# YuemingJin/STswinCL

Measured on AMD Instinct MI355X. Metric: input frames/s, TswinPlus fwd+bwd+Adam, 4-frame 512x512 clips, higher is better.
Workload: dtype bf16; 1 GPU; BASELINE.json configs[1]: TswinPlus(12) seg train step, 4 clips/GPU x T=4 frames x 3x512x512, swin res (64,64), OHEM-CE, Adam; T=4 because the reference asserts it (swin_512.py:313); clips_per_gpu=4, frames_per_clip=4, parallelism=dp1, graph_requested=True

## Files before the change

include/stswin_hip.h:

```cpp
#ifndef STSWIN_HIP_H
#define STSWIN_HIP_H
#ifdef __cplusplus
extern "C" {
#endif

#define STSWIN_GF_GELU 1
#define STSWIN_GF_RESID 2
#define STSWIN_GF_MUL_DGELU 4
#define STSWIN_GF_OUT_F32 8
#define STSWIN_GF_ACCUM 16
#define STSWIN_GF_RELU 32
#define STSWIN_GF_MUL_R 8192
#define STSWIN_GF_C2_DGELU 16384
#define STSWIN_GF_CS_PARTIAL 32768
#define STSWIN_GF_CS_SQ 65536
#define STSWIN_GF_TAPSKIP (1 << 29)
#define STSWIN_GF_BIG 128
#define STSWIN_GF_MID 512
#define STSWIN_GF_NOPIPE 1024
#define STSWIN_GF_HALF 2048
#define STSWIN_GF_M32PP (1u << 31)
#define STSWIN_GF_W4R (1 << 30)
#define STSWIN_GF_ROT 4096
#define STSWIN_GF_NOBIG 256
// ... 35 lines not shown
                       void* stream);
long stswin_conv3x3_c64_wgrad_scratch(int frames, int H, int W);
int stswin_conv3x3_c64_wgrad(const void* dy, const void* x, float* dw, int tapminor, int accumulate, float* scratch, long scratch_floats,
                             int frames, int H, int W, void* stream);

int stswin_gemm_nt(int dtype, const void* A, long lda, const int* a_rows, const void* B, long ldb, void* C, long ldc,
                   const int* c_rows, void* C2, long ldc2, const float* bias, const void* R, long ldr,
                   const int* r_rows, int M, int N, int Kseg, int S, float scale, int scale_cols, int flags,
                   float* colsum , void* stream);
int stswin_cs_reduce(const float* partials, int M, int N, float* out, void* stream);
#define STSWIN_TN_OVERWRITE (1 << 27)
#define STSWIN_TN_NO_COMBINE (1 << 26)
long stswin_gemm_nt_splitk_scratch(int M, int N, int Kseg, int S);
int stswin_gemm_nt_splitk(const void* A, long lda, const int* a_rows, const void* B, long ldb, void* C, long ldc, const float* bias, int M, int N,
                          int Kseg, int S, int relu, float* workspace, long workspace_floats, void* stream);
int stswin_tn_fused_hold(int delta);
int stswin_set_cu_budget(int cus);
int stswin_gemm_tn(int dtype, const void* At, long lda, const int* at_rows, const void* Bt, long ldb, const int* bt_rows,
                   float* C, long ldc, int Mk, int Ni, int Nj, int splits, int bseg,
                   float* workspace , long workspace_floats, void* stream);
#define STSWIN_TN_GROUP_DECLINED (-1050)
typedef struct stswin_tn_problem {
  const void* At; long lda; const int* at_rows;
  const void* Bt; long ldb; const int* bt_rows;
  float* C; long ldc;
  int Mk, Ni, Nj, bseg;
  int overwrite;
  int tapminor;
} stswin_tn_problem;
int stswin_gemm_tn_group(int dtype, int count, const stswin_tn_problem* problems, float* workspace, long workspace_floats, int* splits_out,
                         void* stream);
int stswin_tn_combine(const float* workspace, float* C, long ldc, int Ni, int Nj, int splits, int overwrite, int slab_bf16,
                      void* stream);
#define STSWIN_VAR_F32 100
#define STSWIN_VAR_NT_RING256_REGEPI 1
#define STSWIN_VAR_NT_RING256_LDSEPI 2
#define STSWIN_VAR_NT_RING256_NOPIPE 3
#define STSWIN_VAR_NT_RING256_W4 14
#define STSWIN_VAR_NT_STREAM 4
#define STSWIN_VAR_NT_DUO 5
#define STSWIN_VAR_NT_RING256x128_PP 6
#define STSWIN_VAR_NT_MID 7
#define STSWIN_VAR_NT_256x64 8
#define STSWIN_VAR_NT_128x64 9
#define STSWIN_VAR_NT_128x128 10
#define STSWIN_VAR_NT_128x128_W4 11
#define STSWIN_VAR_NT_SPLITK 13
#define STSWIN_VAR_NT_ROWS 12
#define STSWIN_VAR_TN_RING_PLAIN 20
#define STSWIN_VAR_TN_RING_ATROWS 21
#define STSWIN_VAR_TN_RING_BTROWS 22
#define STSWIN_VAR_TN_RING_BSEG 23
#define STSWIN_VAR_TN_128x128 30
#define STSWIN_VAR_TN_128x128_W4 31
#define STSWIN_VAR_TN_ROWS 32
#define STSWIN_VAR_TN_SLABS_F32 0x1000
#define STSWIN_VAR_TN_SLABS_BF16 0x2000
#define STSWIN_VAR_TN_FUSED 0x8000
#define STSWIN_VAR_TN_TAPMINOR 0x4000
#define STSWIN_TN_OUT_TAPMINOR (1 << 25)
int stswin_gemm_nt_qkv_fp8(const void* A, long lda, const int* a_rows, const void* B, long ldb, void* out8, long ld8, float* scales,
                           long ld_scales, const float* bias, int M, int N, int Kseg, float scale, int scale_cols, int rows_per_problem,
                           int head_dim, void* stream);
int stswin_win_attn_fwd_f8(const void* qkv8, long ld8, const float* scales, long ld_scales, void* out, long ldo, const float* biasT,
                           const float* maskT, int nB_, int nW, int T_frames, int ws, int heads, int C, int bias_windows,
                           const int* bias_index, void* stream);
// ... 232 lines not shown
```

stswincl_amd/csrc/gemm.hip:

```cpp
#include "common.h"
#include "stswin_hip.h"
#include <cstdint>
#include <cstdlib>
#include <type_traits>

enum {
  GF_GELU = STSWIN_GF_GELU, GF_RESID = STSWIN_GF_RESID, GF_MUL_DGELU = STSWIN_GF_MUL_DGELU, GF_OUT_F32 = STSWIN_GF_OUT_F32,
  GF_ACCUM = STSWIN_GF_ACCUM, GF_RELU = STSWIN_GF_RELU, GF_MUL_R = STSWIN_GF_MUL_R, GF_C2_DGELU = STSWIN_GF_C2_DGELU,
  GF_CS_PARTIAL = STSWIN_GF_CS_PARTIAL, GF_CS_SQ = STSWIN_GF_CS_SQ, GF_TAPSKIP = STSWIN_GF_TAPSKIP,
  GF_WAVES4 = STSWIN_GF_WAVES4, GF_BIG = STSWIN_GF_BIG, GF_NOBIG = STSWIN_GF_NOBIG, GF_MID = STSWIN_GF_MID, GF_NOPIPE = STSWIN_GF_NOPIPE,
  GF_HALF = STSWIN_GF_HALF, GF_ROT = STSWIN_GF_ROT, GF_NOREGEPI = STSWIN_GF_NOREGEPI, GF_NOSTREAM = STSWIN_GF_NOSTREAM,
  GF_DUO = STSWIN_GF_DUO, GF_STREAM = STSWIN_GF_STREAM, GF_NONARROW = STSWIN_GF_NONARROW, GF_NODEEP = STSWIN_GF_NODEEP,
  GF_DEEP = STSWIN_GF_DEEP, GF_W4R = STSWIN_GF_W4R, GF_M32PP = (int)STSWIN_GF_M32PP,
};

#ifdef STSWIN_TUNING
#define STSWIN_DBG(flags, bit) (((flags) & (1 << (bit))) != 0)
#else
#define STSWIN_DBG(flags, bit) false
#endif
enum { GF_DEBUG_BITS = (1 << 17) | (1 << 18) | (1 << 19) | (1 << 20) | (1 << 21) };
#ifdef STSWIN_TUNING
static __device__ int g_dbg_stagger[2] = {8, 0};
extern "C" int stswin_debug_set_stagger(int phases, int ticks) {
// ... 1600 lines not shown
      for (int u = 0; u < 8; ++u) v[u] = *(const bf16x8*)(src + (long)(s + u) * total);
#pragma unroll
      for (int u = 0; u < 8; ++u)
#pragma unroll
        for (int e = 0; e < 8; ++e) a[e] += (float)v[u][e];
    }
    for (; s < splits; ++s) {
      const bf16x8 v = *(const bf16x8*)(src + (long)s * total);
#pragma unroll
      for (int e = 0; e < 8; ++e) a[e] += (float)v[e];
    }
    if (perm > 0) {
      const int S = Nj / perm, sg = j / perm, c = j - sg * perm;
      float* d = C + (long)i * ldc + (long)c * S + sg;
#pragma unroll
      for (int e = 0; e < 8; ++e) d[(long)e * S] = overwrite ? a[e] : d[(long)e * S] + a[e];
      return;
    }
    float* dst = C + (long)i * ldc + j;
    if ((ldc & 3) == 0) {
      f32x4 lo = {a[0], a[1], a[2], a[3]}, hi = {a[4], a[5], a[6], a[7]};
      if (!overwrite) { lo += *(const f32x4*)dst; hi += *(const f32x4*)(dst + 4); }
      *(f32x4*)dst = lo;
      *(f32x4*)(dst + 4) = hi;
    } else {
      for (int e = 0; e < 8; ++e) dst[e] = overwrite ? a[e] : dst[e] + a[e];
    }
    return;
  }
  const long idx = ((long)blockIdx.x * 256 + threadIdx.x) * 4;
  if (idx >= (long)Ni * Nj) return;
  const int i = idx / Nj, j = idx % Nj;
  f32x4 a = {0.f, 0.f, 0.f, 0.f};
  for (int s = 0; s < splits; ++s) a += *(const f32x4*)(slabs + (long)s * Ni * Nj + idx);
  if (perm > 0) {
    const int S = Nj / perm, sg = j / perm, c = j - sg * perm;
    float* d = C + (long)i * ldc + (long)c * S + sg;
#pragma unroll
    for (int e = 0; e < 4; ++e) d[(long)e * S] = overwrite ? a[e] : d[(long)e * S] + a[e];
    return;
  }
  float* dst = C + (long)i * ldc + j;
  if (overwrite) {
    if ((ldc & 3) == 0) *(f32x4*)dst = a;
    else { for (int e = 0; e < 4; ++e) dst[e] = a[e]; }
  } else if ((ldc & 3) == 0) { *(f32x4*)dst = *(const f32x4*)dst + a; }
  else { for (int e = 0; e < 4; ++e) dst[e] += a[e]; }
}

static thread_local int g_last_variant[2] = {0, 0};
extern "C" int stswin_tuning_build() {
#ifdef STSWIN_TUNING
  return 1;
#else
  return 0;
#endif
}
extern "C" int stswin_last_variant(int family) { return family >= 0 && family < 2 ? g_last_variant[family] : -1; }

static int set_lds_once(const void* fn) {
  return (int)hipFuncSetAttribute(fn, hipFuncAttributeMaxDynamicSharedMemorySize, 65536);
}

extern "C" int stswin_cs_reduce(const float* partials, int M, int N, float* out, void* stream) {
  if (M <= 0 || N <= 0) return 0;
  if (N % 4) return -1004;
  const int rows = 2 * ((M + 255) / 256);
// ... 716 lines not shown
  dim3 grid(((Ni + 127) / 128) * ((Nj + 127) / 128) * splits);
  static int once = set_lds_once((const void*)gemm_tn_kernel<bf16, 4>) | set_lds_once((const void*)gemm_tn_kernel<float, 4>) |
                    set_lds_once((const void*)gemm_tn_kernel<bf16, 8>) | set_lds_once((const void*)gemm_tn_kernel<float, 8>);
  (void)once;
  const bool w8 = splits_flags_w4 == 0;
  g_last_variant[1] = ((w8 ? STSWIN_VAR_TN_128x128 : STSWIN_VAR_TN_128x128_W4) + (dtype ? STSWIN_VAR_F32 : 0)) |
                      (use_slabs ? (slab_bf16 ? STSWIN_VAR_TN_SLABS_BF16 : STSWIN_VAR_TN_SLABS_F32) : 0) | ((use_slabs && perm) ? 0x4000 : 0) |
                      (splits << 16);
  if (dtype == 0) {
    if (w8) hipLaunchKernelGGL((gemm_tn_kernel<bf16, 8>), grid, dim3(512), 65536, (hipStream_t)stream, p);
    else hipLaunchKernelGGL((gemm_tn_kernel<bf16, 4>), grid, dim3(256), 65536, (hipStream_t)stream, p);
  } else {
    if (w8) hipLaunchKernelGGL((gemm_tn_kernel<float, 8>), grid, dim3(512), 65536, (hipStream_t)stream, p);
    else hipLaunchKernelGGL((gemm_tn_kernel<float, 4>), grid, dim3(256), 65536, (hipStream_t)stream, p);
  }
  if (use_slabs && !no_combine) {
    const long n4 = slab_bf16 ? ((long)Ni * Nj + 7) / 8 : ((long)Ni * Nj + 3) / 4;
    hipLaunchKernelGGL(tn_reduce_kernel, dim3((unsigned)((n4 + 255) / 256)), dim3(256), 0, (hipStream_t)stream, workspace, C, ldc,
                       Ni, Nj, splits, overwrite, slab_bf16, perm);
  }
  STSWIN_CHECK_LAUNCH();
  return 0;
}

extern "C" int stswin_tn_combine(const float* workspace, float* C, long ldc, int Ni, int Nj, int splits, int overwrite, int slab_bf16,
                                 void* stream) {
  if (!workspace || !C || Ni <= 0 || Nj <= 0 || splits < 2) return -1007;
  const long n4 = slab_bf16 ? ((long)Ni * Nj + 7) / 8 : ((long)Ni * Nj + 3) / 4;
  hipLaunchKernelGGL(tn_reduce_kernel, dim3((unsigned)((n4 + 255) / 256)), dim3(256), 0, (hipStream_t)stream, workspace, C, ldc, Ni, Nj,
                     splits, overwrite, slab_bf16, 0);
  STSWIN_CHECK_LAUNCH();
  return 0;
}
```

stswincl_amd/headops.py:

```python
from __future__ import annotations

import os
import weakref
from typing import List, Optional, Sequence, Tuple

import torch
import torch.nn.functional as F

from . import hip
from .ops import compute_dtype, _f32

KGRAN = 64


_INDEX_MAPS = {}
_TORCH_PADVEC = os.environ.get("STSWIN_TORCH_PADVEC") == "1"
_BN_KEEP_Y = os.environ.get("STSWIN_BN_KEEP_Y") == "1"


class Layout:

    def __init__(self, segs: Sequence[Tuple[int, int, int]], width: int):
        self.segs, self.width = list(segs), width
        self.logical = sum(s[1] for s in self.segs)
# ... 140 lines not shown
        if ctx.halo:
            hip.conv3x3_c64(X, _conv_mats(weight, dt, lin, lout, False), y, frames, Hin, Win, 1, stats_out=tab)
        else:
            hip.gemm_nt(X, _conv_mats(weight, dt, lin, lout, False), y, M=Mo, a_rows=fmap, S=k * k,
                        bias=lout.pad_vec(bias) if bias is not None else None, stats_out=tab, flags=ctx.tapskip)
        ctx.geom = (frames, Hin, Win)
        ctx.cfg = (k, lin, lout, dt, x.dtype, bias is not None, Mi, Mo)
        ctx.save_for_backward(X, weight, fmap, imap)
        if want_stats:
            ctx.mark_non_differentiable(tab)
            ctx.set_materialize_grads(False)
            return y, tab
        return y

    @staticmethod
    @hip.tn_deferred_backward
    def backward(ctx, dy, _dtab=None):
        if dy is None:
            return (None,) * 8
        X, weight, fmap, imap = ctx.saved_tensors
        k, lin, lout, dt, in_dtype, has_bias, Mi, Mo = ctx.cfg
        co, ci = weight.shape[:2]
        S = k * k
        g = dy.detach().to(dt).contiguous()
        from .ops import wgrad_buffer
        dense = lin.is_identity and lout.is_identity
        direct = dense and S == 1
        dwp = (wgrad_buffer(weight, (lout.width, S * lin.width), X.device) if dense
               else torch.empty(lout.width, S * lin.width, dtype=torch.float32, device=X.device))
        if ctx.halo and _HALO_WGRAD and hip.conv3x3_c64_wgrad_ok(*ctx.geom):
            hip.conv3x3_c64_wgrad(g, X, dwp, *ctx.geom, tapminor=True)
            tapminor = True
        else:
            hip.gemm_tn(g, X, dwp, Mk=Mo, bt_rows=fmap, bseg=lin.width if fmap is not None else 0, overwrite=True,
                        tapminor=dense and S > 1)
            tapminor = dense and S > 1 and hip.last_tn_tapminor()
        dx = None
        if ctx.needs_input_grad[0]:
            dx = torch.empty(Mi, lin.width, dtype=dt, device=X.device)
            pend = ctx.link.take(dt, dx.shape) if ctx.link is not None else None
            if ctx.halo:
                hip.conv3x3_c64(g, _conv_mats(weight, dt, lin, lout, True), dx, *ctx.geom, -1, resid=pend)
            else:
                hip.gemm_nt(g, _conv_mats(weight, dt, lin, lout, True), dx, M=Mi, a_rows=imap, S=S, resid=pend,
                            flags=(hip.GF_RESID if pend is not None else 0) | ctx.tapskip)
            dx = dx.to(in_dtype)
            if ctx.link is not None and not ctx.link.last():
                ctx.link.put(dx)
                dx = None
        hip.tn_join()
        if direct or tapminor:
            dw = dwp
        elif dense:
            dw = dwp.clone().view(co, S, ci).permute(0, 2, 1)
        else:
            dw = torch.zeros(co, ci, S, dtype=torch.float32, device=X.device)
            d3 = dwp.view(lout.width, S, lin.width)
            for oa, on, ob in lout.segs:
                for ia, in_, ib in lin.segs:
                    dw[oa:oa + on, ia:ia + in_, :] = d3[ob:ob + on, :, ib:ib + in_].permute(0, 2, 1)
        db = None
        if has_bias:
            dbp = hip.zeros(lout.width, device=X.device)
            hip.colsum(g, dbp)
            db = lout.unpad_vec(dbp)
        if dw is dwp:
            dw = dw.view(co, ci, k, k)
        else:
            dw = dw.reshape(co, ci, k, k)
# ... 79 lines not shown

    @staticmethod
    def forward(ctx, img, weight, dt, want_stats=False):
        F_, _, Hh, Ww = img.shape
        Ho, Wo = (Hh + 6 - 7) // 2 + 1, (Ww + 6 - 7) // 2 + 1
        im = img.detach().float().contiguous()
        A, Hs, Ws = hip.stem_s2d(im, dt)
        rmap = _stem_rowmap(F_, Ho, Wo, Hs, Ws, img.device)
        y = torch.empty(F_ * Ho * Wo, 64, dtype=dt, device=img.device)
        tab = hip.stats_table(y.shape[0], 64, img.device) if want_stats else None
        if _STEM_CONV and hip.stem_wgrad_ok(Hh, Ww, dt):
            hip.stem_conv(A, _stem_pack(weight, dt), y, F_, Hh, Ww, stats_out=tab)
        else:
            hip.gemm_nt(A, _stem_pack(weight, dt), y, M=y.shape[0], a_rows=rmap, S=4, stats_out=tab)
        ctx.dt, ctx.geom = dt, (F_, Hh, Ww)
        ctx.save_for_backward(A, rmap, weight)
        if want_stats:
            ctx.mark_non_differentiable(tab)
            ctx.set_materialize_grads(False)
            return y, tab
        return y

    @staticmethod
    @hip.tn_deferred_backward
    def backward(ctx, dy, _dtab=None):
        if dy is None:
            return None, None, None, None
        A, rmap, weight = ctx.saved_tensors
        dw = torch.empty(64, 256, dtype=torch.float32, device=A.device)
        g = dy.detach().to(ctx.dt).contiguous()
        if _STEM_WGRAD and hip.stem_wgrad_ok(ctx.geom[1], ctx.geom[2], ctx.dt):
            hip.stem_wgrad(g, A, dw, *ctx.geom)
        else:
            hip.gemm_tn(g, A, dw, Mk=rmap.shape[1], bt_rows=rmap, bseg=64, overwrite=True)
            hip.tn_join()
        dwv = _stem_unpack(dw)
        from .dp import grad_dest
        dest = grad_dest(weight) if getattr(weight, "_stswin_grad_dest", None) is not None else None
        return None, (dest.copy_(dwv) if dest is not None else dwv.contiguous()), None, None


def stem_conv_tokens(img, weight, dt, stats=False):
    F_, _, Hh, Ww = img.shape
    M = F_ * ((Hh - 1) // 2 + 1) * ((Ww - 1) // 2 + 1)
    if stats and _FUSED_BN_STATS and dt == torch.bfloat16 and M >= 8192 and M % 256 == 0:
        return StemConvFn.apply(img, weight, dt, True)
    return StemConvFn.apply(img, weight, dt), None


class MaxPoolTokFn(torch.autograd.Function):

    @staticmethod
    def forward(ctx, x, geom):
        frames, Hh, Ww = geom
        dt = compute_dtype(x)
        X = x.detach().to(dt).contiguous()
        Ho, Wo = (Hh + 2 - 3) // 2 + 1, (Ww + 2 - 3) // 2 + 1
        y = torch.empty(frames * Ho * Wo, X.shape[1], dtype=dt, device=x.device)
        arg = torch.empty(frames * Ho * Wo, X.shape[1], dtype=torch.uint8, device=x.device)
        hip.maxpool3x3s2(X, y, arg, frames, Hh, Ww, Ho, Wo)
        ctx.cfg = (frames, Hh, Ww, Ho, Wo, dt, x.dtype)
        ctx.save_for_backward(arg)
        return y

    @staticmethod
    def backward(ctx, dy):
        (arg,) = ctx.saved_tensors
# ... 607 lines not shown
```

stswincl_amd/hip.py:

```python
from __future__ import annotations

import ctypes
import functools
import os
import re
from typing import Optional

import torch

_ROOT = os.path.dirname(os.path.dirname(os.path.abspath(__file__)))
LIB_PATH = os.environ.get("STSWIN_HIP_LIB") or os.path.join(_ROOT, "stswincl_amd", "lib", "libstswin_hip.so")
HEADER_PATH = os.path.join(_ROOT, "include", "stswin_hip.h")
_lib: Optional[ctypes.CDLL] = None

_c_int, _c_float, _c_void_p = ctypes.c_int, ctypes.c_float, ctypes.c_void_p


class StswinHipError(RuntimeError):
    pass


_C_TYPES = {"int": ctypes.c_int, "long": ctypes.c_long, "float": ctypes.c_float, "double": ctypes.c_double}


# ... 636 lines not shown
    if tapminor and bseg > 0:
        splits |= TN_OUT_TAPMINOR
    Ni, Nj = out_f32.shape
    assert out_f32.dtype == torch.float32 and At.dtype == Bt.dtype
    ws = None if atomics or torch.cuda.is_current_stream_capturing() and At.device not in _TN_WS else _tn_workspace(At.device)
    name = "gemm_tn_bf16" if At.dtype == torch.bfloat16 else "gemm_tn_f32"
    if _SHAPE_NAMES:
        name += f" Mk={Mk} Ni={Ni} Nj={Nj} bseg={bseg} a={int(at_rows is not None)} b={int(bt_rows is not None)}"
    defer = _TN_DEFER > 0 and _TN_DEFER_ON and ws is not None and not debug_ts
    tn_join()
    with _Span(name, 2.0 * Mk * Ni * Nj):
        rc = load().stswin_gemm_tn(_dt(At), _p(At), _ld(At), _p(at_rows), _p(Bt), _ld(Bt),
                                   _p(bt_rows), _p(out_f32), (-1 if debug_ts is True else -int(debug_ts)) if debug_ts else _ld(out_f32), Mk, Ni, Nj,
                                   (splits | TN_NO_COMBINE) if defer else splits, bseg, _p(ws),
                                   ws.numel() if ws is not None else 0, _stream())
    _check(rc, "gemm_tn")
    _log_variant("tn", (Mk, Ni, Nj, bseg), 1)
    if defer:
        v = load().stswin_last_variant(1)
        if v & (VAR_TN_SLABS_F32 | VAR_TN_SLABS_BF16):
            global _TN_PENDING
            cur = torch.cuda.current_stream()
            side = _TN_SIDE.get(At.device)
            if side is None:
                side = _TN_SIDE[At.device] = torch.cuda.Stream(device=At.device)
            ev = torch.cuda.Event()
            ev.record(cur)
            side.wait_event(ev)
            _check(load().stswin_tn_combine(_p(ws), _p(out_f32), _ld(out_f32), Ni, Nj, v >> 16, 1 if (splits & TN_OVERWRITE) else 0,
                                            1 if v & VAR_TN_SLABS_BF16 else 0, side.cuda_stream), "tn_combine")
            _TN_PENDING = torch.cuda.Event()
            _TN_PENDING.record(side)
    return out_f32


class _TnProblem(ctypes.Structure):
    _fields_ = [("At", ctypes.c_void_p), ("lda", ctypes.c_long), ("at_rows", ctypes.c_void_p),
                ("Bt", ctypes.c_void_p), ("ldb", ctypes.c_long), ("bt_rows", ctypes.c_void_p),
                ("C", ctypes.c_void_p), ("ldc", ctypes.c_long),
                ("Mk", ctypes.c_int), ("Ni", ctypes.c_int), ("Nj", ctypes.c_int), ("bseg", ctypes.c_int),
                ("overwrite", ctypes.c_int), ("tapminor", ctypes.c_int)]


LAST_TN_GROUP_SPLITS: list = []


def gemm_tn_group(problems) -> bool:
    n = len(problems)
    if n == 0:
        return True
    first = problems[0]["At"]
    if n > 4 or first.dtype != torch.bfloat16 or torch.cuda.is_current_stream_capturing() and first.device not in _TN_WS:
        return False
    arr = (_TnProblem * n)()
    flops = 0.0
    for i, q in enumerate(problems):
        At, Bt, out = q["At"], q["Bt"], q["out"]
        assert out.dtype == torch.float32 and At.dtype == Bt.dtype == torch.bfloat16
        ar, br = q.get("at_rows"), q.get("bt_rows")
        arr[i] = _TnProblem(At.data_ptr(), _ld(At), ar.data_ptr() if ar is not None else None, Bt.data_ptr(), _ld(Bt),
                            br.data_ptr() if br is not None else None, out.data_ptr(), _ld(out), q["Mk"], out.shape[0], out.shape[1],
                            q.get("bseg", 0), 1 if q.get("overwrite", True) else 0, 1 if q.get("tapminor", False) else 0)
        flops += 2.0 * q["Mk"] * out.shape[0] * out.shape[1]
    ws = _tn_workspace(first.device)
    tn_join()
    sp = (_c_int * n)()
# ... 1535 lines not shown
```

stswincl_amd/ops.py:

```python
from __future__ import annotations

import os
import weakref
from typing import Dict, Optional, Tuple

import torch

from . import hip

_ROWMAPS: Dict[tuple, torch.Tensor] = {}
_WCACHE: Dict[tuple, tuple] = {}


def compute_dtype(x: torch.Tensor) -> torch.dtype:
    if x.dtype == torch.bfloat16 or x.dtype == torch.float16:
        return torch.bfloat16
    if torch.is_autocast_enabled():
        return torch.bfloat16
    return torch.float32


def window_rowmap(B, T, H, W, ws, shift, device) -> torch.Tensor:
    key = ("win", B, T, H, W, ws, shift, str(device))
    m = _ROWMAPS.get(key)
# ... 375 lines not shown
    @staticmethod
    @hip.tn_deferred_backward
    def backward(ctx, dout):
        (X2, rmap, qkv, biasT, maskT, o, x1, mean2, rstd2, n2, h_pre, h, y2, mean1, rstd1,
         qkv_w, proj_w, n1_w, n2_w, fc1_w, fc2_w, index, qscale) = ctx.saved_tensors
        H, W, ws, shift, heads = ctx.geom
        dt = ctx.dt
        M, C = rmap.numel(), X2.shape[1]
        N, d = ws * ws, C // heads
        nW = (H // ws) * (W // ws)
        dev = X2.device
        hid = fc1_w.shape[0]
        tsz = (2 * ws - 1) * (2 * ws - 1)
        (dn1_w, dn1_b, dfc2_b, dfc1_b, dn2_w, dn2_b, dproj_b, dbiasT, dqkv_b, dtable) = zeros_like_list(
            [(C,), (C,), (C,), (hid,), (C,), (C,), (C,), (heads, N, N), (3 * C,), (tsz, heads)], dev)
        dfc2_w, dfc1_w, dproj_w, dqkv_w = (wgrad_buffer(fc2_w, (C, hid), dev), wgrad_buffer(fc1_w, (hid, C), dev),
                                           wgrad_buffer(proj_w, (C, C), dev), wgrad_buffer(qkv_w, (3 * C, C), dev))
        g = dout.detach().to(dt).contiguous().view(M, C)
        folds = hip.deferred_folds()
        folds.__enter__()
        try:
            dy2 = hip.layernorm_bwd(g, y2, _f32(n1_w), mean1, rstd1, dn1_w, dn1_b, M=M, dxsum=dfc2_b)
            late = [dict(At=dy2, Bt=h, out=dfc2_w, Mk=M)]
            dh_pre = torch.empty(M, hid, dtype=dt, device=dev)
            hip.gemm_nt(dy2, wcast(fc2_w, dt, True), dh_pre, M=M, resid=h_pre,
                        flags=(hip.GF_MUL_DGELU if ctx.gelu_bwd else hip.GF_MUL_R) | _duo("fc2d", M, hid, C), colsum_out=dfc1_b)
            late.append(dict(At=dh_pre, Bt=n2, out=dfc1_w, Mk=M))
            dn2 = torch.empty(M, C, dtype=dt, device=dev)
            hip.gemm_nt(dh_pre, wcast(fc1_w, dt, True), dn2, M=M)
            del dh_pre
            if _TN_GROUP:
                dx1 = hip.layernorm_bwd(dn2, x1, _f32(n2_w), mean2, rstd2, dn2_w, dn2_b, M=M, add=dy2, dxsum=dproj_b)
            else:
                hip.gemm_tn(dy2, h, dfc2_w, Mk=M, overwrite=True)
                late.pop(0)
                dx1 = hip.layernorm_bwd(dn2, x1, _f32(n2_w), mean2, rstd2, dn2_w, dn2_b, M=M, dx=dy2, accumulate=True,
                                        dxsum=dproj_b)
            late.append(dict(At=dx1, Bt=o, out=dproj_w, Mk=M, at_rows=rmap))
            do = dn2
            hip.gemm_nt(dx1, wcast(proj_w, dt, True), do, M=M, a_rows=rmap, colsum_out=dqkv_b[2 * C:])
            if qscale is not None:
                dqkv = hip.win_attn_bwd_f8(qkv, qscale, do, biasT, maskT, dbiasT, nB_=(M // (2 * N)), nW=nW, T=2, ws=ws, heads=heads,
                                           C=C, scale=d ** -0.5, colsum_out=dqkv_b, bias_index=ctx.bidx)
            else:
                dqkv = hip.win_attn_bwd(qkv, do, biasT, maskT, dbiasT, nB_=(M // (2 * N)), nW=nW, T=2, ws=ws, heads=heads,
                                        C=C, scale=d ** -0.5, colsum_out=dqkv_b, bias_index=ctx.bidx)
        except BaseException:
            folds.abort()
            raise
        folds.__exit__(None, None, None)
        hip.bias_scatter(dbiasT, index.reshape(-1).contiguous(), dtable, N, heads, lists=_scatter_lists_for(index, ws, tsz))
        late.append(dict(At=dqkv, Bt=X2, out=dqkv_w, Mk=M, bt_rows=rmap if ctx.src is None else ctx.src.compose(rmap)))

        def single(q):
            hip.gemm_tn(q["At"], q["Bt"], q["out"], Mk=M, at_rows=q.get("at_rows"), bt_rows=q.get("bt_rows"), overwrite=True)
        if not (_TN_GROUP and len(late) == 4 and _TN_GROUP4 and hip.gemm_tn_group(late)):
            if len(late) == 4:
                single(late.pop(0))
            if not (_TN_GROUP and hip.gemm_tn_group(late)):
                for q in late:
                    single(q)
        del late
        src = ctx.src
        if src is None:
            dx = torch.empty(M, C, dtype=dt, device=dev)
            hip.gemm_nt(dqkv, wcast(qkv_w, dt, True), dx, M=M, c_rows=rmap, resid=dx1, r_rows=rmap, flags=hip.GF_RESID)
            Bp = M // (2 * H * W)
            dx_ret = dx.view(Bp, 2, H * W, C).to(ctx.in_dtype)
        else:
            dx, mine = src.grad_buffer(X2.shape, dt, dev)
            hip.gemm_nt(dqkv, wcast(qkv_w, dt, True), dx, M=M, c_rows=src.compose(rmap), resid=dx1, r_rows=rmap, flags=hip.GF_RESID)
            dx_ret = dx.view(ctx.x_shape).to(ctx.in_dtype) if mine else None
        return (dx_ret, dqkv_w, dqkv_b, dtable, dproj_w, dproj_b, dn1_w, dn1_b,
                dn2_w, dn2_b, dfc1_w, dfc1_b, dfc2_w, dfc2_b, None, None, None, None, None)


class PatchMergeFn(torch.autograd.Function):

    @staticmethod
    def forward(ctx, x, norm_w, norm_b, red_w, res):
        H, W = res
        dt = compute_dtype(x)
        B, T, L, C = x.shape
        assert T == 4, "wrong time dimension"
        assert L == H * W, "input feature has wrong size"
        assert H % 2 == 0 and W % 2 == 0, f"x size ({H}*{W}) are not even."
        frames = B * T
        M4 = frames * (H // 2) * (W // 2)
        X2 = x.detach().to(dt).contiguous().view(frames * L, C)
        rows = merge_rowmap(frames, H, W, x.device)
        n, mean, rstd = hip.layernorm_fwd(X2, _f32(norm_w), _f32(norm_b), M=M4, rows=rows, S=4, Cseg=C)
        y = torch.empty(M4, 2 * C, dtype=dt, device=x.device)
        hip.gemm_nt(n, wcast(red_w, dt), y, M=M4)
        ctx.res, ctx.dt, ctx.in_dtype, ctx.shape = res, dt, x.dtype, (B, T, L, C)
        ctx.save_for_backward(X2, rows, n, mean, rstd, norm_w, red_w)
        return y.view(B, T, L // 4, 2 * C)

    @staticmethod
    @hip.tn_deferred_backward
    def backward(ctx, dy):
        X2, rows, n, mean, rstd, norm_w, red_w = ctx.saved_tensors
        B, T, L, C = ctx.shape
        dt = ctx.dt
        M4 = n.shape[0]
        dev = X2.device
        g = dy.detach().to(dt).contiguous().view(M4, 2 * C)
        dred = wgrad_buffer(red_w, (2 * C, 4 * C), dev)
        hip.gemm_tn(g, n, dred, Mk=M4, overwrite=True)
        dn = torch.empty(M4, 4 * C, dtype=dt, device=dev)
        hip.gemm_nt(g, wcast(red_w, dt, True), dn, M=M4)
        dg = hip.zeros(4 * C, device=dev)
        db = hip.zeros(4 * C, device=dev)
        dx = torch.empty_like(X2)
        hip.layernorm_bwd(dn, X2, _f32(norm_w), mean, rstd, dg, db, M=M4, rows=rows, S=4, Cseg=C, dx=dx)
        return dx.view(B, T, L, C).to(ctx.in_dtype), dg, db, dred, None


class WindowAttentionFn(torch.autograd.Function):

    @staticmethod
    def forward(ctx, x, qkv_w, qkv_b, table, proj_w, proj_b, index, mask, ws, heads):
        dt = compute_dtype(x)
        B_, T, N, C = x.shape
        M, d = B_ * T * N, C // heads
        nW = mask.shape[0] if mask is not None else 1
        X2 = x.detach().to(dt).contiguous().view(M, C)
        qkv = torch.empty(M, 3 * C, dtype=dt, device=x.device)
        hip.gemm_nt(X2, wcast(qkv_w, dt), qkv, M=M, bias=_f32(qkv_b), scale=d ** -0.5, scale_cols=C)
        biasT = hip.bias_expand(_f32(table), index.reshape(-1).contiguous(), None, N, heads)
        maskT = mask.detach().float().transpose(1, 2).contiguous() if mask is not None else None
        o = hip.win_attn_fwd(qkv, biasT, maskT, nB_=B_, nW=nW, T=T, ws=ws, heads=heads, C=C)
        y = torch.empty(M, C, dtype=dt, device=x.device)
        hip.gemm_nt(o, wcast(proj_w, dt), y, M=M, bias=_f32(proj_b))
        ctx.cfg = (ws, heads, nW, T)
        ctx.dt, ctx.in_dtype = dt, x.dtype
        ctx.save_for_backward(X2, qkv, biasT, maskT, o, qkv_w, proj_w, index)
        return y.view(B_, T, N, C)

    @staticmethod
    @hip.tn_deferred_backward
    def backward(ctx, dy):
        X2, qkv, biasT, maskT, o, qkv_w, proj_w, index = ctx.saved_tensors
        ws, heads, nW, T = ctx.cfg
        dt = ctx.dt
        M, C = X2.shape
        N, d = ws * ws, C // heads
        dev = X2.device
        z = lambda *s: torch.zeros(*s, dtype=torch.float32, device=dev)
        g = dy.detach().to(dt).contiguous().view(M, C)
        dproj_w, dproj_b = z(C, C), z(C)
        hip.gemm_tn(g, o, dproj_w, Mk=M)
        hip.colsum(g, dproj_b)
        do = torch.empty(M, C, dtype=dt, device=dev)
        hip.gemm_nt(g, wcast(proj_w, dt, True), do, M=M)
        dbiasT = z(heads, N, N)
        dqkv = hip.win_attn_bwd(qkv, do, biasT, maskT, dbiasT, nB_=M // (T * N), nW=nW, T=T, ws=ws, heads=heads, C=C,
                                scale=d ** -0.5)
        dtable = z((2 * ws - 1) * (2 * ws - 1), heads)
        hip.bias_scatter(dbiasT, index.reshape(-1).contiguous(), dtable, N, heads)
        dqkv_w, dqkv_b = z(3 * C, C), z(3 * C)
        hip.gemm_tn(dqkv, X2, dqkv_w, Mk=M)
        hip.colsum(dqkv, dqkv_b)
        dx = torch.empty(M, C, dtype=dt, device=dev)
        hip.gemm_nt(dqkv, wcast(qkv_w, dt, True), dx, M=M)
        return (dx.view(M // (T * N), T, N, C).to(ctx.in_dtype), dqkv_w, dqkv_b, dtable, dproj_w, dproj_b,
                None, None, None, None)


class LinearFn(torch.autograd.Function):

    @staticmethod
    def forward(ctx, x, w, b, act):
        dt = compute_dtype(x)
        K = x.shape[-1]
        X2 = x.detach().to(dt).contiguous().view(-1, K)
        M = X2.shape[0]
        y = torch.empty(M, w.shape[0], dtype=dt, device=x.device)
        pre = torch.empty_like(y) if act == "gelu" else None
        flags = hip.GF_GELU if act == "gelu" else (hip.GF_RELU if act == "relu" else 0)
        hip.gemm_nt(X2, wcast(w, dt), y, M=M, bias=_f32(b), out2=pre, flags=flags)
        ctx.act, ctx.dt, ctx.in_dtype, ctx.has_b = act, dt, x.dtype, b is not None
        ctx.save_for_backward(X2, w, pre if act == "gelu" else (y if act == "relu" else None))
        return y.view(*x.shape[:-1], w.shape[0])

    @staticmethod
    @hip.tn_deferred_backward
    def backward(ctx, dy):
        X2, w, aux = ctx.saved_tensors
        dt = ctx.dt
        M, K = X2.shape
        Nn = w.shape[0]
        g = dy.detach().to(dt).contiguous().view(M, Nn)
        if ctx.act == "relu":
            g = g * (aux > 0).to(dt)
        dx = torch.empty(M, K, dtype=dt, device=X2.device)
        if ctx.act == "gelu":
            dpre = (g.float() * _dgelu(aux.float())).to(dt)
            g = dpre
        dw = wgrad_buffer(w, (Nn, K), X2.device)
        hip.gemm_tn(g, X2, dw, Mk=M, overwrite=True)
        db = None
        if ctx.has_b:
            db = hip.zeros(Nn, device=X2.device)
            hip.colsum(g, db)
        hip.gemm_nt(g, wcast(w, dt, True), dx, M=M)
        return dx.view(*dy.shape[:-1], K).to(ctx.in_dtype), dw, db, None


def _dgelu(x: torch.Tensor) -> torch.Tensor:
    return 0.5 * (1 + torch.erf(x * 0.7071067811865476)) + x * torch.exp(-0.5 * x * x) * 0.3989422804014327
```

Baseline: 621.0 frames/s.

## Add narrow-tile split-K TN GEMM for weight gradients and route wgrads through it

Adds a dedicated split-K weight-gradient GEMM kernel that uses tile shapes suited to outputs with one narrow dimension (at most 128). It uses a 4-stage global-to-LDS pipeline, prefetches row-index maps into LDS, and picks splits from the CU budget, with a per-split slab reduction afterwards. Python routing sends eligible weight-gradient calls (large Mk, narrow Ni or Nj) to this kernel and falls back to the existing gemm_tn otherwise. The slab reduce kernel is also unrolled to batch loads across splits. The intent is better CU occupancy on the skinny wgrad GEMMs in the swin blocks and heads, at the cost of extra slab traffic and another reduce launch.

```diff
diff --git a/include/stswin_hip.h b/include/stswin_hip.h
--- a/include/stswin_hip.h
+++ b/include/stswin_hip.h
@@ -91,6 +91,10 @@
                          void* stream);
 int stswin_tn_combine(const float* workspace, float* C, long ldc, int Ni, int Nj, int splits, int overwrite, int slab_bf16,
                       void* stream);
+long stswin_gemm_tn_narrow_scratch(int Mk, int Ni, int Nj);
+int stswin_gemm_tn_narrow(int dtype, const void* At, long lda, const int* at_rows, const void* Bt, long ldb, const int* bt_rows,
+                          float* C, long ldc, int Mk, int Ni, int Nj, int splits, int bseg, float* workspace, long workspace_floats,
+                          void* stream, int* splits_out);
 #define STSWIN_VAR_F32 100
 #define STSWIN_VAR_NT_RING256_REGEPI 1
 #define STSWIN_VAR_NT_RING256_LDSEPI 2
diff --git a/stswincl_amd/csrc/gemm.hip b/stswincl_amd/csrc/gemm.hip
--- a/stswincl_amd/csrc/gemm.hip
+++ b/stswincl_amd/csrc/gemm.hip
@@ -1656,7 +1656,24 @@
   if (idx >= (long)Ni * Nj) return;
   const int i = idx / Nj, j = idx % Nj;
   f32x4 a = {0.f, 0.f, 0.f, 0.f};
-  for (int s = 0; s < splits; ++s) a += *(const f32x4*)(slabs + (long)s * Ni * Nj + idx);
+  const float* src = slabs + idx;
+  const long total = (long)Ni * Nj;
+  int s = 0;
+  for (; s + 16 <= splits; s += 16) {
+    f32x4 v[16];
+#pragma unroll
+    for (int u = 0; u < 16; ++u) v[u] = *(const f32x4*)(src + (long)(s + u) * total);
+#pragma unroll
+    for (int u = 0; u < 16; ++u) a += v[u];
+  }
+  for (; s + 4 <= splits; s += 4) {
+    f32x4 v[4];
+#pragma unroll
+    for (int u = 0; u < 4; ++u) v[u] = *(const f32x4*)(src + (long)(s + u) * total);
+#pragma unroll
+    for (int u = 0; u < 4; ++u) a += v[u];
+  }
+  for (; s < splits; ++s) a += *(const f32x4*)(src + (long)s * total);
   if (perm > 0) {
     const int S = Nj / perm, sg = j / perm, c = j - sg * perm;
     float* d = C + (long)i * ldc + (long)c * S + sg;
@@ -2439,3 +2456,263 @@
   STSWIN_CHECK_LAUNCH();
   return 0;
 }
+
+template <int RB> DEVI int swz_rb(int row) {
+  if constexpr (RB == 128) return (((row >> 1) & 1) | (((row >> 3) & 1) << 1)) << 1;
+  else return swz256(row);
+}
+template <int RB> DEVI bf16x4 lds_tr4_rb(const char* tile, int k0, int col0) {
+  const int lam = threadIdx.x & 15;
+  const int row = k0 + (lam >> 2), col = col0 + 4 * (lam & 3);
+  const int chunk = (col >> 3) ^ swz_rb<RB>(row);
+  const char* addr = tile + row * RB + (chunk << 4) + ((col & 7) << 1);
+  short4v r = __builtin_amdgcn_ds_read_tr16_b64_v4i16((__attribute__((address_space(3))) short4v*)addr);
+  return __builtin_bit_cast(bf16x4, r);
+}
+
+DEVI void glds4_raw(const void* gsrc, void* lds_wave_base) {
+  const unsigned lds = (unsigned)(unsigned long)(__attribute__((address_space(3))) char*)lds_wave_base;
+  asm volatile("s_mov_b32 m0, %1\n\ts_nop 0\n\tglobal_load_lds_dword %0, off" ::"v"(gsrc), "s"(lds) : "memory", "m0");
+}
+template <int N> DEVI void wait_vmcnt_n() { asm volatile("s_waitcnt vmcnt(%0)" ::"n"(N) : "memory"); }
+
+template <int BI, int BJ, int NW, int WR, int MODE>
+__global__ __launch_bounds__(NW * 64) void gemm_tn_narrow_kernel(GemmTN p) {
+  constexpr int WC = NW / WR, WTJ = BJ / WC, FI = 4, FJ = WTJ / 16;
+  constexpr int NST = 4, KS = 32;
+  constexpr int RBA = BI * 2, RBB = BJ * 2;
+  constexpr int RPIA = 1024 / RBA, RPIB = 1024 / RBB;
+  constexpr int CPRA = RBA / 16, CPRB = RBB / 16;
+  constexpr int NIA = BI / 16 / NW, NIB = BJ / 16 / NW;
+  constexpr int RW = KS / NW;
+  constexpr int D = NIA + NIB;
+  constexpr int ABYTES = KS * RBA, SLOT = KS * (RBA + RBB);
+  constexpr int NTAP = BJ / 64;
+  static_assert(BI / WR == 64 && FJ >= 1 && NIA * RPIA == RW && NIB * RPIB == RW && NIA >= 1 && NIB >= 1, "tile / wave layout");
+  extern __shared__ __attribute__((aligned(16))) char smem[];
+  const int l = threadIdx.x & 63, w = wave_id();
+  const int wr = w / WC, wc = w % WC;
+  const int split_id = blockIdx.x % p.splits, panel = blockIdx.x / p.splits;
+  const int panels_j = (p.Nj + BJ - 1) / BJ;
+  const int i0 = (panel / panels_j) * BI, j0 = (panel % panels_j) * BJ;
+  const int units = (p.Mk + KS - 1) / KS;
+  const int per = (units + p.splits - 1) / p.splits;
+  const int s_begin = split_id * per;
+  const int nt = min(units, s_begin + per) - s_begin;
+  if (nt <= 0) return;
+
+  const char* zero = (const char*)g_stswin_zero;
+  const int rsa = l / CPRA, cpa = l % CPRA, rsb = l / CPRB, cpb = l % CPRB;
+  const int tapbase = p.bseg > 0 ? j0 / p.bseg : 0;
+  const int taps_all = p.bseg > 0 ? p.Nj / p.bseg : 1;
+  int aoff[NIA], boff[NIB], btap[NIB];
+#pragma unroll
+  for (int i = 0; i < NIA; ++i) {
+    const int r = (w * NIA + i) * RPIA + rsa;
+    const int gi = i0 + (cpa ^ swz_rb<RBA>(r)) * 8;
+    aoff[i] = gi < p.Ni ? gi * 2 : -1;
+  }
+#pragma unroll
+  for (int i = 0; i < NIB; ++i) {
+    const int r = (w * NIB + i) * RPIB + rsb;
+    const int gj = j0 + (cpb ^ swz_rb<RBB>(r)) * 8;
+    const int t = p.bseg > 0 ? gj / p.bseg : 0;
+    btap[i] = t - tapbase;
+    boff[i] = gj < p.Nj ? (gj - t * p.bseg) * 2 : -1;
+  }
+  int arow[NIA], brow[NIB];
+  constexpr bool MAP_A = (MODE & 1) != 0, MAP_B = (MODE & 2) != 0;
+  constexpr int DI = (MAP_A ? NIA : 0) + (MAP_B ? NIB : 0);
+  constexpr int NIX = 8;
+  static_assert(2 * D + 3 * DI <= 63, "vmcnt");
+  char* const ixw = smem + NST * SLOT + w * (NIX * DI * 256);
+  long btapoff[NIB];
+#pragma unroll
+  for (int i = 0; i < NIB; ++i) btapoff[i] = p.bseg > 0 ? (long)min(tapbase + btap[i], taps_all - 1) * p.Mk : 0;
+  auto row_a = [&](int s, int i) { return (s_begin + s) * KS + (w * NIA + i) * RPIA + rsa; };
+  auto row_b = [&](int s, int i) { return (s_begin + s) * KS + (w * NIB + i) * RPIB + rsb; };
+  auto issue_idx = [&](int s) {
+    if constexpr (DI > 0) {
+      char* dst = ixw + (s & (NIX - 1)) * (DI * 256);
+      int n = 0;
+      if constexpr (MAP_A) {
+#pragma unroll
+        for (int i = 0; i < NIA; ++i) glds4_raw(p.at_rows + min(row_a(s, i), p.Mk - 1), dst + (n++) * 256);
+      }
+      if constexpr (MAP_B) {
+#pragma unroll
+        for (int i = 0; i < NIB; ++i) glds4_raw(p.bt_rows + btapoff[i] + min(row_b(s, i), p.Mk - 1), dst + (n++) * 256);
+      }
+    }
+  };
+  auto get_rows = [&](int s) {
+    const int* src = (const int*)(ixw + (s & (NIX - 1)) * (DI * 256)) + l;
+    int n = 0;
+#pragma unroll
+    for (int i = 0; i < NIA; ++i) {
+      const int m = row_a(s, i);
+      int v = m;
+      if constexpr (MAP_A) v = src[(n++) * 64];
+      arow[i] = m < p.Mk ? v : -1;
+    }
+#pragma unroll
+    for (int i = 0; i < NIB; ++i) {
+      const int m = row_b(s, i);
+      int v = m;
+      if constexpr (MAP_B) v = src[(n++) * 64];
+      brow[i] = m < p.Mk ? v : -1;
+    }
+  };
+  auto issue = [&](int slot) {
+    char* Ab = smem + slot * SLOT;
+    char* Bb = Ab + ABYTES;
+#pragma unroll
+    for (int i = 0; i < NIA; ++i) {
+      const char* sa = (arow[i] >= 0 && aoff[i] >= 0) ? (const char*)p.At + (long)arow[i] * p.lda * 2 + aoff[i] : zero;
+      glds16_raw(sa, Ab + (w * NIA + i) * 1024);
+    }
+#pragma unroll
+    for (int i = 0; i < NIB; ++i) {
+      const char* sb = (brow[i] >= 0 && boff[i] >= 0) ? (const char*)p.Bt + (long)brow[i] * p.ldb * 2 + boff[i] : zero;
+      glds16_raw(sb, Bb + (w * NIB + i) * 1024);
+    }
+  };
+
+  f32x4 acc[FI][FJ];
+#pragma unroll
+  for (int i = 0; i < FI; ++i)
+#pragma unroll
+    for (int j = 0; j < FJ; ++j) acc[i][j] = (f32x4){0.f, 0.f, 0.f, 0.f};
+  const int fr = l & 15, fq = l >> 4;
+  const bool active = i0 + wr * 64 < p.Ni && j0 + wc * WTJ < p.Nj;
+
+  if constexpr (DI > 0) {
+    issue_idx(0); issue_idx(1); issue_idx(2); issue_idx(3);
+    wait_vmcnt_n<0>();
+  }
+  get_rows(0); issue(0); issue_idx(4);
+  if (nt > 1) { get_rows(1); issue(1); }
+  issue_idx(5);
+  if (nt > 2) { get_rows(2); issue(2); }
+  issue_idx(6);
+  for (int k = 0; k < nt; ++k) {
+    const int newer = min(NST - 2, nt - 1 - k);
+    if (newer >= 2) wait_vmcnt_n<2 * D + 3 * DI>();
+    else if (newer == 1) wait_vmcnt_n<D + 3 * DI>();
+    else wait_vmcnt_n<3 * DI>();
+    asm volatile("s_waitcnt lgkmcnt(0)" ::: "memory");
+    __builtin_amdgcn_s_barrier();
+    asm volatile("" ::: "memory");
+    if (k + NST - 1 < nt) { get_rows(k + NST - 1); issue((k + NST - 1) & (NST - 1)); }
+    issue_idx(k + NST + 3);
+    if (active) {
+      const char* Ab = smem + (k & (NST - 1)) * SLOT;
+      const char* Bb = Ab + ABYTES;
+      bf16x8 a[FI], b[FJ];
+#pragma unroll
+      for (int j = 0; j < FJ; ++j)
+        b[j] = cat4(lds_tr4_rb<RBB>(Bb, 8 * fq, wc * WTJ + j * 16), lds_tr4_rb<RBB>(Bb, 8 * fq + 4, wc * WTJ + j * 16));
+#pragma unroll
+      for (int i = 0; i < FI; ++i)
+        a[i] = cat4(lds_tr4_rb<RBA>(Ab, 8 * fq, wr * 64 + i * 16), lds_tr4_rb<RBA>(Ab, 8 * fq + 4, wr * 64 + i * 16));
+#pragma unroll
+      for (int i = 0; i < FI; ++i)
+#pragma unroll
+        for (int j = 0; j < FJ; ++j) acc[i][j] = __builtin_amdgcn_mfma_f32_16x16x32_bf16(b[j], a[i], acc[i][j], 0, 0, 0);
+    }
+  }
+  wait_vmcnt_n<0>();
+  if (!active) return;
+  float* slab = p.slabs + (long)split_id * p.Ni * p.Nj;
+#pragma unroll
+  for (int i = 0; i < FI; ++i)
+#pragma unroll
+    for (int j = 0; j < FJ; ++j) {
+      const int gi = i0 + wr * 64 + i * 16 + fr;
+      const int gj = j0 + wc * WTJ + j * 16 + 4 * fq;
+      if (gi < p.Ni && gj < p.Nj) *(f32x4*)(slab + (long)gi * p.Nj + gj) = acc[i][j];
+    }
+}
+
+struct TnNarrowPlan { int kind, BI, BJ, lds, tiles, units, splits; };
+static bool tn_narrow_plan(int Mk, int Ni, int Nj, TnNarrowPlan* o) {
+  if (Mk <= 0 || Ni <= 0 || Nj <= 0 || (Ni > 128 && Nj > 128)) return false;
+  const bool a_narrow = Ni <= 128 && (Nj > 128 || Ni <= Nj);
+  if (a_narrow) { o->kind = Ni <= 64 ? 1 : 2; o->BI = Ni <= 64 ? 64 : 128; o->BJ = 256; }
+  else { o->kind = Nj <= 64 ? 4 : 3; o->BI = Nj <= 64 ? 128 : 256; o->BJ = Nj <= 64 ? 64 : 128; }
+  o->lds = 4 * 32 * 2 * (o->BI + o->BJ);
+  o->tiles = ((Ni + o->BI - 1) / o->BI) * ((Nj + o->BJ - 1) / o->BJ);
+  o->units = (Mk + 31) / 32;
+  long s = (long)stswin_cu_budget() / o->tiles;
+  if (s > o->units / 4) s = o->units / 4;
+  const long cap = (long)Mk * (Ni + Nj) / (4L * Ni * Nj);
+  if (s > cap) s = cap;
+  if (s < 1) s = 1;
+  if (s >= 8) s &= ~7L;
+  o->splits = (int)s;
+  return true;
+}
+static int tn_no_empty_split(int units, int splits) {
+  if (splits > units) splits = units;
+  if (splits < 1) splits = 1;
+  const int per = (units + splits - 1) / splits;
+  return (units + per - 1) / per;
+}
+
+extern "C" long stswin_gemm_tn_narrow_scratch(int Mk, int Ni, int Nj) {
+  TnNarrowPlan pl;
+  if (Ni % 8 || Nj % 8 || !tn_narrow_plan(Mk, Ni, Nj, &pl)) return 0;
+  return (long)tn_no_empty_split(pl.units, pl.splits) * Ni * Nj;
+}
+
+template <int BI, int BJ, int NW, int WR, int MODE>
+static void tn_narrow_launch_mode(const GemmTN& q, int tiles, hipStream_t stream) {
+  constexpr int DI = ((MODE & 1) ? BI / 16 / NW : 0) + ((MODE & 2) ? BJ / 16 / NW : 0);
+  constexpr int LDS = 4 * 32 * 2 * (BI + BJ) + NW * 8 * DI * 256;
+  static_assert(LDS <= 163840, "LDS");
+  static int once = (int)hipFuncSetAttribute((const void*)gemm_tn_narrow_kernel<BI, BJ, NW, WR, MODE>, hipFuncAttributeMaxDynamicSharedMemorySize, LDS);
+  (void)once;
+  hipLaunchKernelGGL((gemm_tn_narrow_kernel<BI, BJ, NW, WR, MODE>), dim3((unsigned)(tiles * q.splits)), dim3(NW * 64), LDS, stream, q);
+}
+template <int BI, int BJ, int NW, int WR>
+static void tn_narrow_launch(const GemmTN& q, int tiles, hipStream_t stream) {
+  switch ((q.at_rows ? 1 : 0) | (q.bt_rows ? 2 : 0)) {
+    case 0: tn_narrow_launch_mode<BI, BJ, NW, WR, 0>(q, tiles, stream); break;
+    case 1: tn_narrow_launch_mode<BI, BJ, NW, WR, 1>(q, tiles, stream); break;
+    case 2: tn_narrow_launch_mode<BI, BJ, NW, WR, 2>(q, tiles, stream); break;
+    default: tn_narrow_launch_mode<BI, BJ, NW, WR, 3>(q, tiles, stream); break;
+  }
+}
+
+extern "C" int stswin_gemm_tn_narrow(int dtype, const void* At, long lda, const int* at_rows, const void* Bt, long ldb, const int* bt_rows,
+                                     float* C, long ldc, int Mk, int Ni, int Nj, int splits, int bseg, float* workspace,
+                                     long workspace_floats, void* stream, int* splits_out) {
+  if (splits_out) *splits_out = 0;
+  if (splits < 0) splits = 0;
+  const int overwrite = (splits & STSWIN_TN_OVERWRITE) ? 1 : 0;
+  const int perm = ((splits & STSWIN_TN_OUT_TAPMINOR) && bseg > 0) ? bseg : 0;
+  const int req = splits & ~(STSWIN_TN_OVERWRITE | STSWIN_TN_OUT_TAPMINOR);
+  if (req & ~0xFFFFFF) return -1106;
+  if (dtype != 0) return -1101;
+  TnNarrowPlan pl;
+  if (!At || !Bt || !C || Mk > 0x7FFF0000 || !tn_narrow_plan(Mk, Ni, Nj, &pl)) return -1102;
+  if (Ni % 8 || Nj % 8 || lda % 8 || ldb % 8 || lda < 0 || ldb < 0 || ((unsigned long)At & 15) || ((unsigned long)Bt & 15)) return -1103;
+  if (bseg < 0 || (bseg > 0 && (!bt_rows || bseg % 64 || pl.BJ % bseg || Nj % bseg))) return -1104;
+  if (!workspace || ((unsigned long)workspace & 15) || workspace_floats < (long)Ni * Nj) return -1105;
+  int s = tn_no_empty_split(pl.units, req > 0 ? req : pl.splits);
+  while ((long)s * Ni * Nj > workspace_floats) s = tn_no_empty_split(pl.units, s - 1);
+  if ((long)pl.tiles * s > 0x7FFFFFFFL || (long)Ni * Nj > 0x7FFFFFFFL) return -1102;
+  GemmTN q{At, lda, at_rows, Bt, ldb, bt_rows, C, ldc, Mk, Ni, Nj, s, bseg, workspace, 0, nullptr, overwrite, perm};
+  switch (pl.kind) {
+    case 1: tn_narrow_launch<64, 256, 4, 1>(q, pl.tiles, (hipStream_t)stream); break;
+    case 2: tn_narrow_launch<128, 256, 8, 2>(q, pl.tiles, (hipStream_t)stream); break;
+    case 3: tn_narrow_launch<256, 128, 8, 4>(q, pl.tiles, (hipStream_t)stream); break;
+    default: tn_narrow_launch<128, 64, 4, 2>(q, pl.tiles, (hipStream_t)stream); break;
+  }
+  const long n4 = ((long)Ni * Nj + 3) / 4;
+  hipLaunchKernelGGL(tn_reduce_kernel, dim3((unsigned)((n4 + 255) / 256)), dim3(256), 0, (hipStream_t)stream, workspace, C, ldc, Ni, Nj, s,
+                     overwrite, 0, perm);
+  STSWIN_CHECK_LAUNCH();
+  if (splits_out) *splits_out = s;
+  return 0;
+}
diff --git a/stswincl_amd/headops.py b/stswincl_amd/headops.py
--- a/stswincl_amd/headops.py
+++ b/stswincl_amd/headops.py
@@ -196,9 +196,8 @@
             hip.conv3x3_c64_wgrad(g, X, dwp, *ctx.geom, tapminor=True)
             tapminor = True
         else:
-            hip.gemm_tn(g, X, dwp, Mk=Mo, bt_rows=fmap, bseg=lin.width if fmap is not None else 0, overwrite=True,
-                        tapminor=dense and S > 1)
-            tapminor = dense and S > 1 and hip.last_tn_tapminor()
+            tapminor = hip.gemm_tn_routed(g, X, dwp, Mk=Mo, bt_rows=fmap, bseg=lin.width if fmap is not None else 0, overwrite=True,
+                                          tapminor=dense and S > 1)
         dx = None
         if ctx.needs_input_grad[0]:
             dx = torch.empty(Mi, lin.width, dtype=dt, device=X.device)
@@ -344,7 +343,7 @@
         if _STEM_WGRAD and hip.stem_wgrad_ok(ctx.geom[1], ctx.geom[2], ctx.dt):
             hip.stem_wgrad(g, A, dw, *ctx.geom)
         else:
-            hip.gemm_tn(g, A, dw, Mk=rmap.shape[1], bt_rows=rmap, bseg=64, overwrite=True)
+            hip.gemm_tn_routed(g, A, dw, Mk=rmap.shape[1], bt_rows=rmap, bseg=64, overwrite=True)
             hip.tn_join()
         dwv = _stem_unpack(dw)
         from .dp import grad_dest
diff --git a/stswincl_amd/hip.py b/stswincl_amd/hip.py
--- a/stswincl_amd/hip.py
+++ b/stswincl_amd/hip.py
@@ -692,6 +692,52 @@
             _TN_PENDING = torch.cuda.Event()
             _TN_PENDING.record(side)
     return out_f32
+
+
+_TN_NARROW = os.environ.get("STSWIN_NO_TN_NARROW") != "1"
+LAST_TN_NARROW_SPLITS = [0]
+
+
+def tn_narrow_routed(Mk: int, Ni: int, Nj: int, bseg: int = 0) -> bool:
+    if not _TN_NARROW or Mk < 2048 or min(Ni, Nj) > 128:
+        return False
+    return not (Ni > 128 and Nj > 64)
+
+
+def gemm_tn_narrow(At: torch.Tensor, Bt: torch.Tensor, out_f32: torch.Tensor, *, Mk: int, at_rows=None, bt_rows=None, splits: int = 0,
+                   bseg: int = 0, overwrite: bool = False, tapminor: bool = False) -> bool:
+    Ni, Nj = out_f32.shape
+    assert out_f32.dtype == torch.float32 and At.dtype == Bt.dtype
+    if torch.cuda.is_current_stream_capturing() and At.device not in _TN_WS:
+        return False
+    ws = _tn_workspace(At.device)
+    bits = (TN_OVERWRITE if overwrite else 0) | (TN_OUT_TAPMINOR if tapminor and bseg > 0 else 0)
+    name = "gemm_tn_narrow_bf16"
+    if _SHAPE_NAMES:
+        name += f" Mk={Mk} Ni={Ni} Nj={Nj} bseg={bseg} a={int(at_rows is not None)} b={int(bt_rows is not None)}"
+    tn_join()
+    sp = _c_int(0)
+    with _Span(name, 2.0 * Mk * Ni * Nj) as span:
+        rc = load().stswin_gemm_tn_narrow(_dt(At), _p(At), _ld(At), _p(at_rows), _p(Bt), _ld(Bt), _p(bt_rows), _p(out_f32), _ld(out_f32),
+                                          Mk, Ni, Nj, int(splits) | bits, bseg, _p(ws), ws.numel(), _stream(), ctypes.byref(sp))
+        if -1106 <= rc <= -1101:
+            span.cancel()
+    if -1106 <= rc <= -1101:
+        return False
+    _check(rc, "gemm_tn_narrow")
+    LAST_TN_NARROW_SPLITS[0] = int(sp.value)
+    _log_variant("tn_narrow", (Mk, Ni, Nj, bseg), 1)
+    return True
+
+
+def gemm_tn_routed(At: torch.Tensor, Bt: torch.Tensor, out_f32: torch.Tensor, *, Mk: int, at_rows=None, bt_rows=None, bseg: int = 0,
+                   overwrite: bool = False, tapminor: bool = False) -> bool:
+    Ni, Nj = out_f32.shape
+    if (At.dtype == torch.bfloat16 and tn_narrow_routed(Mk, Ni, Nj, bseg)
+            and gemm_tn_narrow(At, Bt, out_f32, Mk=Mk, at_rows=at_rows, bt_rows=bt_rows, bseg=bseg, overwrite=overwrite, tapminor=tapminor)):
+        return bool(tapminor and bseg > 0)
+    gemm_tn(At, Bt, out_f32, Mk=Mk, at_rows=at_rows, bt_rows=bt_rows, bseg=bseg, overwrite=overwrite, tapminor=tapminor)
+    return bool(tapminor and bseg > 0 and last_tn_tapminor())
 
 
 class _TnProblem(ctypes.Structure):
diff --git a/stswincl_amd/ops.py b/stswincl_amd/ops.py
--- a/stswincl_amd/ops.py
+++ b/stswincl_amd/ops.py
@@ -431,7 +431,7 @@
             if _TN_GROUP:
                 dx1 = hip.layernorm_bwd(dn2, x1, _f32(n2_w), mean2, rstd2, dn2_w, dn2_b, M=M, add=dy2, dxsum=dproj_b)
             else:
-                hip.gemm_tn(dy2, h, dfc2_w, Mk=M, overwrite=True)
+                hip.gemm_tn_routed(dy2, h, dfc2_w, Mk=M, overwrite=True)
                 late.pop(0)
                 dx1 = hip.layernorm_bwd(dn2, x1, _f32(n2_w), mean2, rstd2, dn2_w, dn2_b, M=M, dx=dy2, accumulate=True,
                                         dxsum=dproj_b)
@@ -452,7 +452,7 @@
         late.append(dict(At=dqkv, Bt=X2, out=dqkv_w, Mk=M, bt_rows=rmap if ctx.src is None else ctx.src.compose(rmap)))
 
         def single(q):
-            hip.gemm_tn(q["At"], q["Bt"], q["out"], Mk=M, at_rows=q.get("at_rows"), bt_rows=q.get("bt_rows"), overwrite=True)
+            hip.gemm_tn_routed(q["At"], q["Bt"], q["out"], Mk=M, at_rows=q.get("at_rows"), bt_rows=q.get("bt_rows"), overwrite=True)
         if not (_TN_GROUP and len(late) == 4 and _TN_GROUP4 and hip.gemm_tn_group(late)):
             if len(late) == 4:
                 single(late.pop(0))
@@ -505,7 +505,7 @@
         dev = X2.device
         g = dy.detach().to(dt).contiguous().view(M4, 2 * C)
         dred = wgrad_buffer(red_w, (2 * C, 4 * C), dev)
-        hip.gemm_tn(g, n, dred, Mk=M4, overwrite=True)
+        hip.gemm_tn_routed(g, n, dred, Mk=M4, overwrite=True)
         dn = torch.empty(M4, 4 * C, dtype=dt, device=dev)
         hip.gemm_nt(g, wcast(red_w, dt, True), dn, M=M4)
         dg = hip.zeros(4 * C, device=dev)
@@ -548,7 +548,7 @@
         z = lambda *s: torch.zeros(*s, dtype=torch.float32, device=dev)
         g = dy.detach().to(dt).contiguous().view(M, C)
         dproj_w, dproj_b = z(C, C), z(C)
-        hip.gemm_tn(g, o, dproj_w, Mk=M)
+        hip.gemm_tn_routed(g, o, dproj_w, Mk=M)
         hip.colsum(g, dproj_b)
         do = torch.empty(M, C, dtype=dt, device=dev)
         hip.gemm_nt(g, wcast(proj_w, dt, True), do, M=M)
@@ -558,7 +558,7 @@
         dtable = z((2 * ws - 1) * (2 * ws - 1), heads)
         hip.bias_scatter(dbiasT, index.reshape(-1).contiguous(), dtable, N, heads)
         dqkv_w, dqkv_b = z(3 * C, C), z(3 * C)
-        hip.gemm_tn(dqkv, X2, dqkv_w, Mk=M)
+        hip.gemm_tn_routed(dqkv, X2, dqkv_w, Mk=M)
         hip.colsum(dqkv, dqkv_b)
         dx = torch.empty(M, C, dtype=dt, device=dev)
         hip.gemm_nt(dqkv, wcast(qkv_w, dt, True), dx, M=M)
@@ -597,7 +597,7 @@
             dpre = (g.float() * _dgelu(aux.float())).to(dt)
             g = dpre
         dw = wgrad_buffer(w, (Nn, K), X2.device)
-        hip.gemm_tn(g, X2, dw, Mk=M, overwrite=True)
+        hip.gemm_tn_routed(g, X2, dw, Mk=M, overwrite=True)
         db = None
         if ctx.has_b:
             db = hip.zeros(Nn, device=X2.device)
```

After: 623.9 frames/s (median of 6 runs). No clear change (+0.5%).
